# kiyo-masui/bitshuffle

Measured on AMD Instinct MI355X. Metric: device-resident GiB/s bitshuffle+LZ4 encode+decode, 4 GiB int16; % HBM roofline, higher is better.
Workload: dtype u8; 1 GPU; bitshuffle+LZ4 encode+decode round trip, 4 GiB int16 G1 correlated noise per GPU, default blocks (4096 elem), device-resident, decoder rebuilds the block index; elem_size=2, block_size=4096, bytes_per_gpu=4294967296, compressed_bytes_rank0=1813937762, parallelism=shard-per-gpu x1

## Files before the change

### bitshuffle_amd/csrc/bshuf_dev.h

```cpp
#pragma once

#include <hip/hip_runtime.h>
#include <stdint.h>

namespace bshuf {

constexpr int kWave = 64;

constexpr int kBlockedMult = 8;
constexpr int kMinMatch = 4;
constexpr int kMfLimit = 12;
constexpr int kLastLiterals = 5;
constexpr int kLz4MinLength = kMfLimit + 1;
constexpr int kU16TableLimit = 65536 + kMfLimit - 1;
constexpr uint32_t kMaxDistance = 65535;

__host__ __device__ inline int lz4_bound(int n) { return n + n / 255 + 16; }

struct Layout {
    int64_t nfull;
    int32_t bs;
    int32_t last;
    int32_t E;
    int64_t nblocks() const { return nfull + (last ? 1 : 0); }
};

// ... 157 lines not shown
    } else {
#pragma unroll
        for (int i = 0; i < EK / 2; i++) {
            const u32x4 v = *(const gbl128c*)(p + 16 * i);
            w[4 * i + 0] = v.x;
            w[4 * i + 1] = v.y;
            w[4 * i + 2] = v.z;
            w[4 * i + 3] = v.w;
        }
    }
}

template <int EK>
__device__ __forceinline__ void store_group(uint8_t* p, const uint32_t (&w)[2 * EK]) {
    if constexpr (EK == 1) {
        *(gbl64*)p = u32x2{w[0], w[1]};
    } else {
#pragma unroll
        for (int i = 0; i < EK / 2; i++)
            *(gbl128*)(p + 16 * i) = u32x4{w[4 * i + 0], w[4 * i + 1], w[4 * i + 2], w[4 * i + 3]};
    }
}

#ifndef BSHUF_TICKET_SHARDS
#define BSHUF_TICKET_SHARDS 8
#endif
constexpr int kTicketShards = BSHUF_TICKET_SHARDS;
constexpr int kTicketStride = 16;
static_assert((kTicketShards & (kTicketShards - 1)) == 0, "shards: a power of two");

struct Tickets {
    uint32_t* ctr;
    int64_t base;
    __device__ __forceinline__ Tickets(uint32_t* set, int64_t first)
        : ctr(set ? set + (blockIdx.x & (kTicketShards - 1)) * kTicketStride : nullptr),
          base(set ? first + gridDim.x + (blockIdx.x & (kTicketShards - 1)) : (int64_t)gridDim.x) {}
    __device__ __forceinline__ uint32_t request(int lane, uint32_t n = 1u) const {
        uint32_t t = 0;
        if (ctr && lane == 0) t = __hip_atomic_fetch_add(ctr, n, __ATOMIC_RELAXED, __HIP_MEMORY_SCOPE_AGENT);
        return t;
    }
    __device__ __forceinline__ int64_t block(uint32_t t, int64_t last, uint32_t k = 0u) const {
        if (!ctr) return last + base;
        const uint32_t v = (uint32_t)__builtin_amdgcn_readfirstlane((int)t) + k;
        return base + (int64_t)kTicketShards * (int64_t)v;
    }
};

}
```

### bitshuffle_amd/csrc/enc_common.h

```cpp
#pragma once

#include "launch.h"

namespace bshuf {

struct EncArgs {
    const uint8_t* in;
    uint8_t* scratch;
    uint64_t* foot;
    int64_t slot;
    Layout L;
    int32_t desc_ok;
    int32_t desc_off;
    const Seg* segs;
    const uint32_t* blk_seg;
    int32_t raw8;
    int64_t blk0;
    uint32_t* tickets;
};

template <int EK>
struct BlockRegs {
    static constexpr int kIters = EK ? 8192 / (kWave * 8 * EK) : 1;
    uint32_t w[kIters][2 * (EK ? EK : 1)];
};

template <int EK>
__device__ __forceinline__ void issue_block_loads(BlockRegs<EK>& R, const uint8_t* src, int P,
                                                  int lane) {
#pragma unroll
    for (int it = 0; it < BlockRegs<EK>::kIters; it++) {
        const int g = it * kWave + lane;
        if (g < P) load_group<EK>(src + (int64_t)g * 8 * EK, R.w[it]);
    }
}

template <int EK>
__device__ __forceinline__ void transpose_regs_to_lds(const BlockRegs<EK>& R, lds8* D, int P,
                                                      int g0, int lane) {
#pragma unroll
    for (int it = 0; it < BlockRegs<EK>::kIters; it++) {
// ... 103 lines not shown
```

### bitshuffle_amd/csrc/launch.h

```cpp
#pragma once

#include <hip/hip_runtime.h>
#include <stddef.h>
#include <stdint.h>

#include <algorithm>

#include "bshuf_dev.h"

namespace bshuf {

bool prof_on();
class ProfScope {
  public:
    ProfScope(const char* name, hipStream_t s);
    ~ProfScope();

  private:
    const char* name_;
    hipStream_t s_;
    void* a_;
};

int tuning_variant();
#ifdef BSHUF_DIAG
int diag_variant();
#endif

constexpr int kPipeSegs = 8;
constexpr int64_t kPipeMinBlocks = 65536;
constexpr int kPipeEvents = kPipeSegs + 2;
constexpr int kNoPipe = 1 << 20;
struct PipeCtx {
    hipStream_t side = nullptr;
    hipEvent_t ev[kPipeEvents] = {};
};
PipeCtx* pipe_ctx(hipStream_t s);
hipError_t stream_after(hipStream_t s, hipStream_t from, hipEvent_t ev);

constexpr size_t kTicketSetBytes = (size_t)kTicketShards * kTicketStride * sizeof(uint32_t);
constexpr int kEncTicketSets = kPipeSegs;
constexpr int kStaticSched = 1 << 24;
constexpr int kTicketSched = 1 << 25;
enum TicketKernel { kTicketsEncode, kTicketsDecode };
bool ticket_sched(TicketKernel k, int64_t block_bytes);

int64_t persistent_grid(const void* fn, int threads, size_t lds, int64_t work);
hipError_t dev_fill(void* p, int v, size_t n, hipStream_t s);
hipError_t stage_upload(const void* host, size_t bytes, void* dev, hipStream_t s);

struct Seg {
    const uint8_t* in;
    uint8_t* out;
    int64_t first;
    int64_t nfull;
    int64_t tail;
    int64_t in_nbytes;
    int64_t chunk0;
    int64_t nchunks;
    int64_t seq0;
    int64_t* result;
    int32_t last;
    int32_t pad_;
};

hipError_t launch_seg_map(const Seg* segs, int nsegs, uint32_t* map, bool chunks, hipStream_t s);

constexpr int kTileGroups = 256;
// ... 75 lines not shown
```

### bitshuffle_amd/csrc/lz4_decode.hip

```cpp
#include <hipcub/hipcub.hpp>

#include <cstdlib>

#include "launch.h"
#include "lds_copy.h"
#include "lz4_scan.h"

namespace bshuf {

namespace {

constexpr int64_t kAmbiguous = -2;
constexpr int64_t kDead = -1;
constexpr int kIdxWinMax = 32768;
constexpr int kIdxCandCap = 512;

#ifdef BSHUF_DIAG
constexpr int kDDiagCopies = 64;
__device__ unsigned long long g_ddiag[kDDiagCopies * 16];
__device__ unsigned long long g_ddiag_bw[4] = {~0ull, 0, 0, 0};
struct DDiag {
    uint64_t t, acc[8];
    uint32_t cnt[8];
    __device__ DDiag() : t(__builtin_amdgcn_s_memtime()) {
        for (int i = 0; i < 8; i++) acc[i] = 0, cnt[i] = 0;
    }
    __device__ __forceinline__ void stamp(int i) {
        const uint64_t n = __builtin_amdgcn_s_memtime();
        acc[i] += n - t;
        t = n;
    }
    __device__ __forceinline__ void count(int i, uint32_t v) { cnt[i] += v; }
    __device__ void flush(int lane) {
        if (lane == 0)
            for (int i = 0; i < 8; i++) {
                atomicAdd(&g_ddiag[(blockIdx.x % kDDiagCopies) * 16 + i], (unsigned long long)acc[i]);
                atomicAdd(&g_ddiag[(blockIdx.x % kDDiagCopies) * 16 + 8 + i], (unsigned long long)cnt[i]);
            }
        if (lane == 0) {
            atomicMin(&g_ddiag_bw[0], (unsigned long long)cnt[3]);
            atomicMax(&g_ddiag_bw[1], (unsigned long long)cnt[3]);
            atomicAdd(&g_ddiag_bw[2], (unsigned long long)cnt[3]);
            atomicAdd(&g_ddiag_bw[3], 1ull);
// ... 552 lines not shown
        }
        dg.stamp(2);
    }
}

struct DecArgs {
    const uint8_t* in;
    int64_t in_nbytes;
    const uint64_t* offs;
    uint8_t* out;
    int64_t* status;
    long long* bad;
    Layout L;
    uint32_t maxlen;
    int32_t cap;
    uint32_t* seq;
    const Seg* segs;
    const uint32_t* blk_seg;
    int32_t stage_off;
    int32_t ip_end;
    int64_t blk0, blk1;
    const int64_t* dlen;
    uint32_t* tickets;
};

__device__ __forceinline__ void resolve_len(DecArgs& a) {
    if (a.dlen) {
        a.in_nbytes = readable_bytes(*a.dlen, a.in_nbytes);
        a.dlen = nullptr;
    }
}

struct BlockLoc {
    const uint8_t* in;
    int64_t in_nbytes;
    uint8_t* out;
    uint32_t* seq;
    long long* bad;
    int m;
    bool last;
};

__device__ __forceinline__ BlockLoc block_loc(const DecArgs& a, int64_t k, int64_t nb, uint32_t s) {
    BlockLoc b;
    if (!a.segs) {
        b.in = a.in;
// ... 369 lines not shown
    }
    const gbl128c* g4 = span_base(a, sp);
    const int nch = span_chunks(a, sp);
    for (int c = lane; c < nch; c += kWave) ((lds128*)Cbuf)[c] = g4[c];
    return sp.loc.seq[sp.o0 / 3 + lane];
}

template <int EK, int VAR>
__global__ __launch_bounds__(64) __attribute__((amdgpu_waves_per_eu((VAR & 512) ? (EK == 0 ? 4 : 5) : 1)))
void k_lz4_decode(DecArgs a, int64_t nb) {
    extern __shared__ __attribute__((aligned(16))) uint8_t smem[];
    const int lane = threadIdx.x;
    const int E = EK ? EK : a.L.E;
    lds8* D = to_lds(smem);
    lds8* Cbuf = to_lds(smem) + a.cap + 16;
    constexpr bool kG = (VAR & 16) != 0;
    constexpr bool kIP = (VAR & 512) != 0;
    auto cbuf_of = [&](const Span& sp) -> lds8* {
        return kIP ? to_lds(smem) + a.ip_end - 16 * span_chunks(a, sp) : Cbuf;
    };
    int64_t blk = a.blk0 + blockIdx.x;
    const int64_t end = a.blk1;
    if (blk >= end) return;
    const Tickets tks(a.tickets, a.blk0);
    const uint32_t tk0 = tks.request(lane, 2u);
    uint32_t tk = tks.request(lane);
    resolve_len(a);

    PayRegsT<kIP ? kPayItersIP : kPayIters> R;
    auto fits = [&](const Span& sp) { return kIP || span_fits(a, sp); };
    Span cur = span_from(a, issue_offs(a, blk, nb, lane), nb);
    uint32_t cur_pos;
    if constexpr (kG) {
        cur_pos = cur.loc.seq[cur.o0 / 3 + lane];
    } else {
        const bool in_regs = fits(cur);
        if (in_regs) issue_pay(R, a, cur, lane);
        cur_pos = land_record(R, in_regs, a, cur, cbuf_of(cur), lane);
    }
    int64_t next = tks.block(tk0, blk);
    int64_t nn = tks.block(tk0, next, 1u);
    Span nxt = {};
    bool nxt_in_regs = false;
    uint32_t pref_pos = 0;
    constexpr bool kTouch = (VAR & 32) != 0;
    Touch t_cur{0u, 0u}, t_nxt{0u, 0u}, t_nxt2{0u, 0u};
    if (next < end) {
        nxt = span_from(a, issue_offs(a, next, nb, lane), nb);
        if constexpr (kG) {
            pref_pos = nxt.loc.seq[nxt.o0 / 3 + lane];
            if constexpr (kTouch) t_nxt = touch_record(nxt, lane);
        } else {
            nxt_in_regs = fits(nxt);
            if (nxt_in_regs) issue_pay(R, a, nxt, lane);
        }
    }
    OffRegs O{0, 0};
    if (nn < end) O = issue_offs(a, nn, nb, lane);
    int64_t n3 = end;
    auto offs_ahead = [&]() {
        n3 = tks.block(tk, nn);
        if (n3 < end) {
            tk = tks.request(lane);
            O = issue_offs(a, n3, nb, lane);
        }
    };
    __builtin_amdgcn_fence(__ATOMIC_RELEASE, "wavefront");
    __builtin_amdgcn_wave_barrier();
    DDiag dg;

    for (;;) {
        dg.stamp(5);
        const int P = cur.loc.m / 8;
        const int cp = span_shift(a, cur);
        lds8* const CB = cbuf_of(cur);
        const lds8* C = CB + cp;
        int status = 0, clen = 0;
        if (cur.scan < 0) {
            status = (int)cur.scan;
        } else if constexpr (kG) {
            if constexpr (kTouch) touch_done(t_cur);
            const uint8_t* rec = cur.loc.in + cur.o0;
            clen = (int)be32_global(rec);
            const uintptr_t b0 = (uintptr_t)(rec + 4);
// ... 147 lines not shown
                    nxt2_in_regs = fits(nxt2);
                    if (nxt2_in_regs) issue_pay(R, a, nxt2, lane);
                }
            }
        }
        __builtin_amdgcn_fence(__ATOMIC_RELEASE, "wavefront");
        __builtin_amdgcn_wave_barrier();
        dg.stamp(4);
        dg.count(3, 1);
        if (next >= end) break;
        blk = next;
        cur = nxt;
        cur_pos = nxt_pos;
        next = nn;
        nn = n3;
        nxt = nxt2;
        nxt_in_regs = nxt2_in_regs;
        if constexpr (kTouch) {
            t_cur = t_nxt;
            t_nxt = t_nxt2;
        }
    }
    dg.flush(lane);
}

__global__ __launch_bounds__(256) void k_decode_finish(const int64_t* __restrict__ status,
                                                       const uint64_t* __restrict__ offs,
                                                       int64_t nblocks, const long long* bad,
                                                       const int64_t* idx_err, const uint8_t* in,
                                                       int64_t in_nbytes, uint8_t* tail_dst,
                                                       int64_t tail, int64_t* result,
                                                       const int64_t* dlen) {
    if (dlen) {
        const int64_t d = *dlen;
        if (d < 0) {
            if (threadIdx.x == 0) *result = d;
            return;
        }
        in_nbytes = readable_bytes(d, in_nbytes);
    }
    const long long last_bad = *bad;
    const int64_t end = nblocks ? (int64_t)offs[nblocks - 1] + status[nblocks - 1] : 0;
    const bool idx_bad = idx_err && *idx_err != 0;
    const bool ok = last_bad < 0 && !idx_bad && end + tail <= in_nbytes;
    if (ok)
        for (int64_t i = threadIdx.x; i < tail; i += blockDim.x) tail_dst[i] = in[end + i];
// ... 258 lines not shown
            if (diag_variant() == 64) fn = BSHUF_DEC(4, 576);
            if (diag_variant() == 72) fn = BSHUF_DEC(4, 584);
#endif
            break;
        case 8: fn = inplace ? BSHUF_DEC(8, 512) : touch ? BSHUF_DEC(8, 48) : (grec ? BSHUF_DEC(8, 16) : BSHUF_DEC(8, 0)); break;
        default: fn = inplace ? BSHUF_DEC(0, 512) : touch ? BSHUF_DEC(0, 48) : (grec ? BSHUF_DEC(0, 16) : BSHUF_DEC(0, 0)); break;
    }
#undef BSHUF_DEC
    hipError_t e = hipSuccess;
#if defined(BSHUF_DIAG) || defined(BSHUF_OCC)
    if (const char* w = getenv("BSHUF_DIAG_DEC_WAVES")) {
        const size_t want = (size_t)(160 * 1024 / atoi(w)) & ~(size_t)1023;
        if (want > lds) lds = want;
    }
#endif
    if (lds > 65536) {
        e = hipFuncSetAttribute(fn, hipFuncAttributeMaxDynamicSharedMemorySize, (int)lds);
        if (e != hipSuccess) return e;
    }
    auto dec = [&](int64_t f0, int64_t f1, hipStream_t st) -> hipError_t {
        DecArgs aa = a;
        aa.blk0 = f0;
        aa.blk1 = f1;
        const dim3 grid((unsigned)persistent_grid(fn, kWave, lds, f1 - f0));
        ProfScope prof("k_lz4_decode", st);
        void* args[] = {&aa, const_cast<int64_t*>(&nb)};
        hipError_t r = hipLaunchKernel(fn, grid, dim3(kWave), args, lds, st);
        return r != hipSuccess ? r : hipGetLastError();
    };
    a.blk0 = 0;
    a.blk1 = nb;
    if (!ticket_sched(kTicketsDecode, (int64_t)L.bs * L.E) || nb >= ((int64_t)1 << 31)) a.tickets = nullptr;
    e = scan_impl(a, nb, s);
    return e != hipSuccess ? e : dec(0, nb, s);
}

__global__ void k_seg_dlen(Seg* __restrict__ segs, const int64_t* __restrict__ dlens, int nsegs) {
    const int i = (int)(blockIdx.x * blockDim.x + threadIdx.x);
    if (i < nsegs) segs[i].in_nbytes = readable_bytes(dlens[i], segs[i].in_nbytes);
}

__global__ __launch_bounds__(64) void k_decode_finish_batch(const int64_t* __restrict__ status,
                                                            const uint64_t* __restrict__ offs,
                                                            const long long* bad,
                                                            const int64_t* idx_err, const Seg* segs,
                                                            int32_t bs, int32_t E, const int64_t* dlens) {
// ... 66 lines not shown
    ProfScope prof("k_decode_finish", s);
    hipLaunchKernelGGL(k_decode_finish_batch, dim3((unsigned)nsegs), dim3(64), 0, s, b.status, b.offs,
                       (const long long*)b.bad, (const int64_t*)b.idx_err, segs, L.bs, L.E, dlens);
    return hipGetLastError();
}

}

#ifdef BSHUF_DIAG
extern "C" int bshuf_diag_read_dec(unsigned long long* out) {
    static unsigned long long all[bshuf::kDDiagCopies * 16];
    if (hipMemcpyFromSymbol(all, HIP_SYMBOL(bshuf::g_ddiag), sizeof all) != hipSuccess) return -1;
    for (int i = 0; i < 16; i++) {
        out[i] = 0;
        for (int c = 0; c < bshuf::kDDiagCopies; c++) out[i] += all[c * 16 + i];
    }
    static const unsigned long long bw0[4] = {~0ull, 0, 0, 0};
    if (hipMemcpyFromSymbol(out + 16, HIP_SYMBOL(bshuf::g_ddiag_bw), sizeof bw0) != hipSuccess ||
        hipMemcpyToSymbol(HIP_SYMBOL(bshuf::g_ddiag_bw), bw0, sizeof bw0) != hipSuccess)
        return -1;
    static const unsigned long long z[bshuf::kDDiagCopies * 16] = {0};
    return hipMemcpyToSymbol(HIP_SYMBOL(bshuf::g_ddiag), z, sizeof z) == hipSuccess ? 0 : -1;
}
#endif
```

### bitshuffle_amd/csrc/lz4_encode.hip

```cpp
#include <hipcub/hipcub.hpp>

#include <atomic>
#include <type_traits>
#include <cstdlib>
#include <mutex>

#include "enc_common.h"
#include "launch.h"
#include "lds_copy.h"

namespace bshuf {

namespace {

constexpr int kTableBytes = 16384;

#ifdef BSHUF_DIAG
constexpr int kDiagCopies = 64;
__device__ unsigned long long g_diag[kDiagCopies * 32];
#define DIAG_DECL                                   \
    uint64_t _dt = __builtin_amdgcn_s_memtime();    \
    uint64_t _acc[8] = {0, 0, 0, 0, 0, 0, 0, 0};    \
    uint32_t _cnt[8] = {0, 0, 0, 0, 0, 0, 0, 0};
#define STAMP(i)                                       \
    do {                                               \
        const uint64_t _n = __builtin_amdgcn_s_memtime(); \
        _acc[i] += _n - _dt;                           \
        _dt = _n;                                      \
    } while (0)
#define COUNT(i, v) (_cnt[i] += (v))
#define DIAG_FLUSH                                                          \
    do {                                                                    \
        if (lane == 0)                                                      \
            for (int _i = 0; _i < 8; _i++) {                                \
                atomicAdd(&g_diag[(blockIdx.x % kDiagCopies) * 32 + _i],   \
                          (unsigned long long)_acc[_i]);                    \
                atomicAdd(&g_diag[(blockIdx.x % kDiagCopies) * 32 + 8 + _i], \
                          (unsigned long long)_cnt[_i]);                    \
            }                                                               \
    } while (0)
__device__ unsigned long long g_diag_bw[4] = {~0ull, 0, 0, 0};
#define KDIAG_DECL                                   \
    uint64_t _kt = __builtin_amdgcn_s_memtime();     \
    uint64_t _kacc[4] = {0, 0, 0, 0};                \
    unsigned long long _kblocks = 0;
#define KBLOCK (++_kblocks)
#define KSTAMP(i)                                       \
    do {                                                \
        const uint64_t _n = __builtin_amdgcn_s_memtime(); \
        _kacc[i] += _n - _kt;                           \
        _kt = _n;                                       \
    } while (0)
#define KDIAG_FLUSH                                                                     \
    do {                                                                                \
        if (lane == 0)                                                                  \
            for (int _i = 0; _i < 4; _i++)                                              \
                atomicAdd(&g_diag[(blockIdx.x % kDiagCopies) * 32 + 16 + _i], _kacc[_i]); \
        if (lane == 0) {                                                                \
            atomicMin(&g_diag_bw[0], _kblocks);                                         \
            atomicMax(&g_diag_bw[1], _kblocks);                                         \
            atomicAdd(&g_diag_bw[2], _kblocks);                                         \
            atomicAdd(&g_diag_bw[3], 1ull);                                             \
        }                                                                               \
    } while (0)
// ... 1500 lines not shown
}
__device__ __forceinline__ void raw_to_lds(const RawRegs& R, lds8* S, int nbytes, int lane) {
#pragma unroll
    for (int it = 0; it < kRawIters; it++) {
        const int i = it * kWave + lane;
        if (8 * i < nbytes) ((lds64v*)S)[i] = u32x2{R.w[it].x, R.w[it].y};
    }
}

#ifndef BSHUF_FLUSH4
#define BSHUF_FLUSH4 1
#endif
template <int EK, bool WIDE, int VAR>
__global__ __launch_bounds__(64) void k_lz4_encode(EncArgs a, int64_t nb) {
    extern __shared__ __attribute__((aligned(16))) uint8_t smem[];
    __builtin_amdgcn_s_setprio(2);
    const int lane = threadIdx.x;
    const int E = EK ? EK : a.L.E;
    (void)smem;
    lds8* const L0 = lds_origin();
    lds8* D = L0 + kTableBytes;
    int64_t blk = blockIdx.x;
    if (blk >= nb) return;
    const Tickets tks(a.tickets, 0);
    uint32_t tk = tks.request(lane);
    constexpr bool kBatch = (VAR & 256) != 0;
    auto blk_m = [&](int64_t k) {
        if (!kBatch) return k < a.L.nfull ? a.L.bs : a.L.last;
        const Seg& g = a.segs[a.blk_seg[k + a.blk0]];
        return k + a.blk0 - g.first < g.nfull ? a.L.bs : g.last;
    };
    auto blk_src = [&](int64_t k) {
        if (!kBatch) return a.in + k * (int64_t)a.L.bs * E;
        const Seg& g = a.segs[a.blk_seg[k + a.blk0]];
        return g.in + (k + a.blk0 - g.first) * (int64_t)a.L.bs * E;
    };

    BlockRegs<EK> R;
    BlockRegs4<EK> R4;
    RawRegs RW;
    auto raw_fits = [&](int m) { return EK == 0 && a.raw8 && m * E <= kRawBytes; };
    constexpr bool kX4 = (VAR & 4) == 0;
    constexpr bool kReadback = (VAR & 128) != 0;
    constexpr int kRegGroups = BlockRegs<EK>::kIters * kWave;
    constexpr int kRegGroups4 = BlockRegs4<EK>::kIters * kWave * 4;
    auto fits = [&](int m) { return EK != 0 && m / 8 <= kRegGroups; };
    auto fits4 = [&](int m) { return kX4 && EK != 0 && (m / 8) % 4 == 0 && m / 8 <= kRegGroups4; };
    if constexpr (EK != 0) {
// ... 92 lines not shown
#pragma unroll
                    for (int it = 0; it < BlockRegs<EK>::kIters; it++) {
                        const int g = g0 + it * kWave + lane;
                        if (g < P) load_group<EK>(src + (int64_t)g * 8 * EK, T.w[it]);
                    }
                    transpose_regs_to_lds<EK>(T, D, P, g0, lane);
                }
            }
        } else {
            for (int i = lane; i < P * E; i += kWave) {
                const int g = i / E, b = i - g * E;
                uint64_t v = 0;
#pragma unroll
                for (int k = 0; k < 8; k++)
                    v |= (uint64_t)src[(int64_t)(8 * g + k) * E + b] << (8 * k);
                v = tr8x8(v);
#pragma unroll
                for (int j = 0; j < 8; j++) D[(8 * b + j) * P + g] = (uint8_t)(v >> (8 * j));
            }
        }
        __builtin_amdgcn_fence(__ATOMIC_RELEASE, "wavefront");
        __builtin_amdgcn_wave_barrier();
        const int64_t next = tks.block(tk, blk);
        if (next < nb) tk = tks.request(lane);
        if constexpr (kDefer) {
            flush_pending();
            if constexpr (kFlush4) {
#pragma unroll
                for (int k = 0; k < kTableBytes / 16 / kWave; k++)
                    ((lds128*)L0)[k * kWave + lane] = u32x4{0u, 0u, 0u, 0u};
            } else {
                for (int i = lane; i < kTableBytes / 16; i += kWave)
                    ((lds128*)L0)[i] = u32x4{0u, 0u, 0u, 0u};
            }
            __builtin_amdgcn_fence(__ATOMIC_RELEASE, "wavefront");
            __builtin_amdgcn_wave_barrier();
        }
        if constexpr (EK != 0) {
            if (next < nb) {
                const int mn = blk_m(next);
                if (fits4(mn))
                    issue_block_loads4<EK>(R4, blk_src(next), mn / 8, lane);
                else if (fits(mn))
                    issue_block_loads<EK>(R, blk_src(next), mn / 8, lane);
            }
        } else {
// ... 34 lines not shown
                    }
                } else {
                    for (int i = lane; i < kTableBytes / 16; i += kWave)
                        ((lds128*)L0)[i] = u32x4{0u, 0u, 0u, 0u};
                    __builtin_amdgcn_fence(__ATOMIC_RELEASE, "wavefront");
                    __builtin_amdgcn_wave_barrier();
                }
            }
        }
        if (c < 0) {
            EmitBytes<> em{out + 4, D, lane};
            c = lz4_encode_block<WIDE, kReadback, (VAR & (8 | 512 | 2048))>(D, n, T, em, lane);
            if (lane < 4) out[lane] = (uint8_t)((uint32_t)c >> (24 - 8 * lane));
        }
        if (lane == 0 && pend_blk != blk) a.foot[blk] = 4 + (uint64_t)c;
        __builtin_amdgcn_fence(__ATOMIC_RELEASE, "wavefront");
        __builtin_amdgcn_wave_barrier();
        KSTAMP(2);
        if (next >= nb) break;
        blk = next;
    }
    if constexpr (kDefer) flush_pending();
    KDIAG_FLUSH;
}

constexpr int kCompactPerWg = 4;
constexpr int kCompactUnroll = 4;

__device__ __forceinline__ u32x4 pair_bytes(const u32x4 a, const u32x4 b, int t) {
    const uint32_t w[8] = {a.x, a.y, a.z, a.w, b.x, b.y, b.z, b.w};
    const uint32_t sh = (uint32_t)(t & 3);
    u32x4 v;
    switch (t >> 2) {
#define BSHUF_PAIR(D)                                                                          \
    case D:                                                                                     \
        v = u32x4{__builtin_amdgcn_alignbyte(w[D + 1], w[D], sh),                               \
                  __builtin_amdgcn_alignbyte(w[D + 2], w[D + 1], sh),                           \
                  __builtin_amdgcn_alignbyte(w[D + 3], w[D + 2], sh),                           \
                  __builtin_amdgcn_alignbyte(w[D + 4], w[D + 3], sh)};                          \
        break;
        BSHUF_PAIR(0)
        BSHUF_PAIR(1)
        BSHUF_PAIR(2)
        default: BSHUF_PAIR(3)
#undef BSHUF_PAIR
    }
// ... 298 lines not shown
                         const EncodeBufs& b, int64_t* d_result, hipStream_t s, bool fast) {
    const int64_t nb = L.nblocks();
    hipError_t e = fill_foot_end(b, nb, s);
    if (e != hipSuccess) return e;
    fast = fast && (int64_t)L.bs * L.E <= kFastMaxBlockBytes;
    if (nb > 0 && (int64_t)L.bs * L.E > max_lds_encode_bytes()) {
        e = launch_encode_large(in, L, b, b.shuf, b.tables, s);
        if (e != hipSuccess) return e;
    } else if (nb > 0) {
        const int64_t nmax = (int64_t)L.bs * L.E;
        const bool wide = nmax >= kU16TableLimit;
        const bool desc = !wide && 4 + lz4_bound((int)nmax) + 15 <= kTableBytes;
        const int32_t desc_off = (int32_t)(((nmax + 15) & ~15) + kDataPad);
        EncArgs a{in, b.scratch, b.foot, b.slot, L, desc ? 1 : 0, desc_off, nullptr, nullptr,
                  ((uintptr_t)in & 7) == 0 ? 1 : 0};
        const size_t lds = kTableBytes + (size_t)desc_off + (desc ? kDescBytes : 0);
        const bool wide_last = L.last && (int64_t)L.last * L.E >= kU16TableLimit;
        const bool aligned = ((uintptr_t)in & 15) == 0;
        const int ek = aligned && (L.E == 1 || L.E == 2 || L.E == 4 || L.E == 8) ? L.E : 0;
        auto go = [&](Layout LL, bool w, int64_t count, int64_t first, int set) -> hipError_t {
            EncArgs aa = a;
            aa.L = LL;
            aa.tickets = ticket_set(b, L, nb, set);
            aa.in = a.in + first * (int64_t)L.bs * L.E;
            aa.scratch = a.scratch + first * b.slot;
            aa.foot = a.foot + first;
            aa.L.nfull = LL.nfull - first;
            if (fast) return launch_encode_fast(aa, count, ek, s);
#define BSHUF_E(EKV)                                                         \
    case EKV:                                                                \
        return w ? launch_enc_t<EKV, true>(aa, count, lds, s)                \
                 : launch_enc_t<EKV, false>(aa, count, lds, s);
            switch (ek) {
                BSHUF_E(0)
                BSHUF_E(1)
                BSHUF_E(2)
                BSHUF_E(4)
                BSHUF_E(8)
            }
#undef BSHUF_E
            return hipErrorInvalidValue;
        };
        PipeCtx* pc = (wide == wide_last || !L.last) && nb >= kPipeMinBlocks ? pipe_ctx(s) : nullptr;
        if (pc) return encode_pipelined(nb, s, pc, b, [&](int64_t f0, int64_t f1, int set) {
            return go(L, wide, f1 - f0, f0, set);
        }, out, nullptr, nullptr, nullptr, [&](hipStream_t st) {
// ... 40 lines not shown
    const int64_t nb = L.nfull;
    hipError_t e = fill_foot_end(b, nb, s);
    if (e != hipSuccess) return e;
    fast = fast && (int64_t)L.bs * L.E <= kFastMaxBlockBytes;
    if (nb > 0) {
        const int64_t nmax = (int64_t)L.bs * L.E;
        const bool wide = nmax >= kU16TableLimit;
        for (int i = 0; i < nsegs; i++)
            if (hsegs[i].last && ((int64_t)hsegs[i].last * L.E >= kU16TableLimit) != wide)
                return hipErrorInvalidValue;
        const bool desc = !wide && 4 + lz4_bound((int)nmax) + 15 <= kTableBytes;
        const int32_t desc_off = (int32_t)(((nmax + 15) & ~15) + kDataPad);
        bool raw8 = true;
        for (int i = 0; i < nsegs; i++) raw8 = raw8 && ((uintptr_t)hsegs[i].in & 7) == 0;
        EncArgs a{nullptr, b.scratch, b.foot, b.slot, L, desc ? 1 : 0, desc_off, segs, blk_seg,
                  raw8 ? 1 : 0};
        const size_t lds = kTableBytes + (size_t)desc_off + (desc ? kDescBytes : 0);
        bool aligned = true;
        for (int i = 0; i < nsegs; i++) aligned = aligned && ((uintptr_t)hsegs[i].in & 15) == 0;
        const int ek = aligned && (L.E == 1 || L.E == 2 || L.E == 4 || L.E == 8) ? L.E : 0;
        auto go = [&](int64_t f0, int64_t f1, int set) -> hipError_t {
            EncArgs aa = a;
            aa.tickets = ticket_set(b, L, nb, set);
            aa.blk0 = f0;
            aa.scratch = a.scratch + f0 * b.slot;
            aa.foot = a.foot + f0;
            const int64_t cnt = f1 - f0;
            if (fast) return launch_encode_fast(aa, cnt, ek, s);
#define BSHUF_E(EKV)                                                                  \
    case EKV:                                                                         \
        return wide ? launch_enc_t<EKV, true, 256>(aa, cnt, lds, s)                   \
                    : launch_enc_t<EKV, false, 256>(aa, cnt, lds, s);
            switch (ek) {
                BSHUF_E(0)
                BSHUF_E(1)
                BSHUF_E(2)
                BSHUF_E(4)
                BSHUF_E(8)
            }
#undef BSHUF_E
            return hipErrorInvalidValue;
        };
        PipeCtx* pc = nb >= kPipeMinBlocks ? pipe_ctx(s) : nullptr;
        if (pc) return encode_pipelined(nb, s, pc, b, go, nullptr, segs, blk_seg, block_offsets,
                                        [&](hipStream_t st) {
            ProfScope prof("k_encode_finish", st);
// ... 34 lines not shown
hipError_t launch_seg_map(const Seg* segs, int nsegs, uint32_t* map, bool chunks, hipStream_t s) {
    if (nsegs <= 0) return hipSuccess;
    hipLaunchKernelGGL(k_seg_map, dim3((unsigned)nsegs), dim3(256), 0, s, segs, map, chunks ? 1 : 0);
    return hipGetLastError();
}

}

#ifdef BSHUF_DIAG
extern "C" int bshuf_diag_read(unsigned long long* out) {
    static unsigned long long all[bshuf::kDiagCopies * 32];
    if (hipMemcpyFromSymbol(all, HIP_SYMBOL(bshuf::g_diag), sizeof all) != hipSuccess) return -1;
    for (int i = 0; i < 32; i++) {
        out[i] = 0;
        for (int c = 0; c < bshuf::kDiagCopies; c++) out[i] += all[c * 32 + i];
    }
    static const unsigned long long bw0[4] = {~0ull, 0, 0, 0};
    if (hipMemcpyFromSymbol(out + 20, HIP_SYMBOL(bshuf::g_diag_bw), sizeof bw0) != hipSuccess ||
        hipMemcpyToSymbol(HIP_SYMBOL(bshuf::g_diag_bw), bw0, sizeof bw0) != hipSuccess)
        return -1;
    static const unsigned long long z[bshuf::kDiagCopies * 32] = {0};
    return hipMemcpyToSymbol(HIP_SYMBOL(bshuf::g_diag), z, sizeof z) == hipSuccess ? 0 : -1;
}
#endif
```

### bitshuffle_amd/csrc/prof.hip

```cpp
#include <hip/hip_runtime.h>

#include <algorithm>
#include <stdio.h>
#include <stdlib.h>
#include <string.h>

#include <map>
#include <mutex>
#include <string>
#include <vector>

#include "launch.h"

namespace bshuf {

namespace {

struct Rec {
    const char* name;
    hipEvent_t a, b;
};

struct Prof {
    std::mutex mu;
// ... 3 lines not shown
    std::vector<hipEvent_t> pool;
    hipEvent_t get() {
        if (!pool.empty()) {
            hipEvent_t e = pool.back();
            pool.pop_back();
            return e;
        }
        hipEvent_t e = nullptr;
        (void)hipEventCreate(&e);
        return e;
    }
};

Prof& P() {
    static Prof* p = new Prof();
    return *p;
}

}

bool prof_on() { return P().on; }

static thread_local int t_variant = 0;
int tuning_variant() { return t_variant & ~(kNoPipe | kStaticSched | kTicketSched); }
constexpr int64_t kDecodeTicketMinBlock = 2048;
bool ticket_sched(TicketKernel k, int64_t block_bytes) {
    if (t_variant & kStaticSched) return false;
    if (t_variant & kTicketSched) return true;
    return k == kTicketsEncode || block_bytes >= kDecodeTicketMinBlock;
}

namespace {
constexpr int kPipeDevices = 16;
struct PipeSet {
    PipeCtx c[kPipeDevices];
    bool bad[kPipeDevices] = {};
    ~PipeSet() {
        for (PipeCtx& x : c) {
            if (!x.side) continue;
            (void)hipStreamSynchronize(x.side);
            for (hipEvent_t& e : x.ev)
                if (e) (void)hipEventDestroy(e);
            (void)hipStreamDestroy(x.side);
        }
    }
};
thread_local PipeSet t_pipe;
}

PipeCtx* pipe_ctx(hipStream_t s) {
    if (t_variant & kNoPipe) return nullptr;
    hipStreamCaptureStatus cap = hipStreamCaptureStatusNone;
// ... 63 lines not shown
    if (!p.on) return;
    std::lock_guard<std::mutex> g(p.mu);
    if (!p.only.empty() && p.only != name) return;
    a_ = p.get();
    (void)hipEventRecord((hipEvent_t)a_, s);
}

ProfScope::~ProfScope() {
    if (!a_) return;
    Prof& p = P();
    std::lock_guard<std::mutex> g(p.mu);
    hipEvent_t b = p.get();
    (void)hipEventRecord(b, s_);
    p.recs.push_back(Rec{name_, (hipEvent_t)a_, b});
}

}

using namespace bshuf;

extern "C" {

int bshuf_set_variant(int v) {
    const int vv = v & ~(kNoPipe | kStaticSched | kTicketSched);
    if (vv != 0 && vv != 2 && vv != 4 && vv != 8 && vv != 16 && vv != 32 && vv != 64 && vv != 128 && vv != 512 && vv != 1024 && vv != 2048 && vv != 4096 && vv != 8192 && vv != 16384 && vv != 24576 && vv != 40960 && vv != 57344 && vv != 65536 && vv != 319488 &&
        vv != 172032 && vv != 450560 &&
        vv != 2793472 && vv != 3072000)
        return -71;
    t_variant = v;
    return 0;
}

#ifdef BSHUF_DIAG
void bshuf_diag_set_ablation(int v) { g_diag_variant = v; }
#endif

void bshuf_prof_enable(int on) {
    Prof& p = P();
    std::lock_guard<std::mutex> g(p.mu);
    p.on = on != 0;
    if (p.on) {
        const size_t want = 4096 + p.recs.size() * 2;
        while (p.pool.size() < want) {
            hipEvent_t e = nullptr;
            if (hipEventCreate(&e) != hipSuccess) break;
            p.pool.push_back(e);
        }
// ... 41 lines not shown
```

### bitshuffle_amd/csrc/scan_host.cpp

```cpp
#include <stdint.h>

#include "lz4_scan.h"

namespace {
struct HostReader {
    const uint8_t* P;
    uint32_t operator()(int p) const { return P[p]; }
};
struct HostOut {
    uint32_t* pos;
    void put(int i, uint32_t v, int op) {
        pos[i] = v;
        (void)op;
    }
};
}

extern "C" int bshuf_hostcheck_scan(const uint8_t* payload, int clen, int n, uint32_t* pos,
                                    int* nseq) {
    HostReader rd{payload};
    HostOut out{pos};
    int cnt = 0;
    const int r = bshuf::scan_block(rd, clen, n, out, cnt);
    *nseq = cnt;
    return r;
}
```

Before: 325.9 GiB/s.

## Add cross-shard ticket stealing to encoder persistent-kernel scheduler

Extends the sharded atomic ticket scheduler so a wave whose home shard is exhausted reads the other shards' counters and steals blocks from the shard with the most remaining work. The intent is to shrink the tail imbalance where some shards finish early while others still hold blocks. It is enabled by default for the encoder when the block is at least 1 KiB, and the decoder uses a non-stealing instantiation. The cost is extra atomic loads and readlane work at the end of each shard, plus some counter overdraw. Diagnostics for per-shard own and stolen counts are added behind a compile flag.

```diff
diff --git a/bitshuffle_amd/csrc/bshuf_dev.h b/bitshuffle_amd/csrc/bshuf_dev.h
--- a/bitshuffle_amd/csrc/bshuf_dev.h
+++ b/bitshuffle_amd/csrc/bshuf_dev.h
@@ -2,6 +2,8 @@
 
 #include <hip/hip_runtime.h>
 #include <stdint.h>
+
+#include "ticket_steal.h"
 
 namespace bshuf {
 
@@ -205,29 +207,130 @@
     }
 }
 
-#ifndef BSHUF_TICKET_SHARDS
-#define BSHUF_TICKET_SHARDS 8
+constexpr int kTicketStride = 16;
+constexpr int64_t kTicketMaxWaves = 4608;
+constexpr int64_t kTicketOverdraw = kTicketMaxWaves * (3 + kTicketShards);
+static_assert(((int64_t)1 << 31) / kTicketShards + 1 + kTicketOverdraw < ((int64_t)1 << 32),
+              "32-bit counters cover every nb < 2^31");
+
+struct Ticket {
+    uint32_t t;
+    int shard;
+};
+
+template <bool STEAL>
+struct TicketsT {
+    uint32_t* set;
+    int64_t g0;
+    int64_t end;
+    int shard;
+    uint32_t dead;
+    bool steal;
+    __device__ __forceinline__ TicketsT(uint32_t* s, int64_t first, int64_t e, bool st)
+        : set(s),
+          g0(s ? first + gridDim.x : (int64_t)gridDim.x),
+          end(e),
+          shard((int)(blockIdx.x & (kTicketShards - 1))),
+          dead(0u),
+          steal(STEAL && st && kTicketShards > 1) {}
+    __device__ __forceinline__ Ticket request(int lane, uint32_t n = 1u) const {
+        uint32_t t = 0;
+        if (set && lane == 0)
+            t = __hip_atomic_fetch_add(set + shard * kTicketStride, n, __ATOMIC_RELAXED, __HIP_MEMORY_SCOPE_AGENT);
+        return Ticket{t, shard};
+    }
+    __device__ __forceinline__ int64_t block(const Ticket& q, int64_t last, uint32_t k = 0u) {
+        if (!set) return last + g0;
+        if constexpr (!STEAL) {
+            const uint32_t v = (uint32_t)__builtin_amdgcn_readfirstlane((int)q.t) + k;
+            return g0 + shard + (int64_t)kTicketShards * (int64_t)v;
+        }
+        if (__builtin_amdgcn_readfirstlane(q.shard) == shard) {
+            const uint32_t v = (uint32_t)__builtin_amdgcn_readfirstlane((int)q.t) + k;
+            const int64_t b = g0 + shard + (int64_t)kTicketShards * (int64_t)v;
+            if (b < end || !steal) return b;
+        }
+        return uni64(steal_block());
+    }
+    static __device__ __forceinline__ int64_t uni64(int64_t x) {
+        const uint32_t lo = (uint32_t)__builtin_amdgcn_readfirstlane((int)(uint32_t)x);
+        const uint32_t hi = (uint32_t)__builtin_amdgcn_readfirstlane((int)(uint32_t)((uint64_t)x >> 32));
+        return (int64_t)(((uint64_t)hi << 32) | lo);
+    }
+    __device__ __forceinline__ int64_t steal_block() {
+        const int lane = threadIdx.x;
+#pragma unroll 1
+        for (int i = 0; i < kTicketShards; i++) {
+            uint32_t left = 0;
+            if (lane < kTicketShards) {
+                const uint32_t drawn =
+                    __hip_atomic_load(set + lane * kTicketStride, __ATOMIC_RELAXED, __HIP_MEMORY_SCOPE_AGENT);
+                left = ticket_remaining(ticket_limit(g0, 0, end, lane), drawn);
+            }
+            uint32_t rem[kTicketShards];
+#pragma unroll
+            for (int c = 0; c < kTicketShards; c++)
+                rem[c] = (dead >> c) & 1u ? 0u : (uint32_t)__builtin_amdgcn_readlane((int)left, c);
+            const int victim = __builtin_amdgcn_readfirstlane(ticket_victim(rem, shard));
+            if (victim < 0) break;
+            uint32_t t = 0;
+            if (lane == 0)
+                t = __hip_atomic_fetch_add(set + victim * kTicketStride, 1u, __ATOMIC_RELAXED,
+                                           __HIP_MEMORY_SCOPE_AGENT);
+            const uint32_t v = (uint32_t)__builtin_amdgcn_readfirstlane((int)t);
+            const int64_t b = g0 + victim + (int64_t)kTicketShards * (int64_t)v;
+            if (b < end) {
+                shard = victim;
+                return b;
+            }
+            dead |= 1u << victim;
+        }
+        return end;
+    }
+};
+
+using Tickets = TicketsT<true>;
+
+#ifdef BSHUF_DIAG
+constexpr int kShardDiagSlots = 16;
+constexpr int kShardDiagWords = 5;
+constexpr int kShardDiagSize = kShardDiagSlots * kTicketShards * kShardDiagWords;
+struct ShardDiag {
+    uint64_t t0;
+    uint32_t own = 1, stolen = 0;
+    int home;
+    __device__ __forceinline__ ShardDiag()
+        : t0(__builtin_amdgcn_s_memrealtime()), home((int)(blockIdx.x & (kTicketShards - 1))) {}
+    template <bool STEAL>
+    __device__ __forceinline__ void drew(const TicketsT<STEAL>& t, int64_t b) {
+        if (b >= t.end) return;
+        if (t.shard == home) own++;
+        else stolen++;
+    }
+    __device__ __forceinline__ void flush(unsigned long long* g, int slot, int lane) const {
+        if (lane != 0) return;
+        unsigned long long* p = g + ((slot % kShardDiagSlots) * kTicketShards + home) * kShardDiagWords;
+        atomicMin(p + 0, (unsigned long long)t0);
+        atomicMax(p + 1, (unsigned long long)__builtin_amdgcn_s_memrealtime());
+        atomicAdd(p + 2, (unsigned long long)own);
+        atomicAdd(p + 3, (unsigned long long)stolen);
+        atomicAdd(p + 4, stolen ? 1ull : 0ull);
+    }
+};
+template <class Sym>
+inline int shard_diag_read(const Sym& sym, unsigned long long* out) {
+    static unsigned long long init[kShardDiagSize];
+    if (hipMemcpyFromSymbol(out, sym, sizeof init) != hipSuccess) return -1;
+    for (int i = 0; i < kShardDiagSize; i++) init[i] = i % kShardDiagWords == 0 ? ~0ull : 0ull;
+    return hipMemcpyToSymbol(sym, init, sizeof init) == hipSuccess ? 0 : -1;
+}
+#define SHARD_DIAG_DECL ShardDiag _sd
+#define SHARD_DIAG_DREW(t, b) _sd.drew(t, b)
+#define SHARD_DIAG_FLUSH(g, slot, lane) _sd.flush(g, slot, lane)
+#else
+#define SHARD_DIAG_DECL ((void)0)
+#define SHARD_DIAG_DREW(t, b) ((void)0)
+#define SHARD_DIAG_FLUSH(g, slot, lane) ((void)0)
 #endif
-constexpr int kTicketShards = BSHUF_TICKET_SHARDS;
-constexpr int kTicketStride = 16;
-static_assert((kTicketShards & (kTicketShards - 1)) == 0, "shards: a power of two");
-
-struct Tickets {
-    uint32_t* ctr;
-    int64_t base;
-    __device__ __forceinline__ Tickets(uint32_t* set, int64_t first)
-        : ctr(set ? set + (blockIdx.x & (kTicketShards - 1)) * kTicketStride : nullptr),
-          base(set ? first + gridDim.x + (blockIdx.x & (kTicketShards - 1)) : (int64_t)gridDim.x) {}
-    __device__ __forceinline__ uint32_t request(int lane, uint32_t n = 1u) const {
-        uint32_t t = 0;
-        if (ctr && lane == 0) t = __hip_atomic_fetch_add(ctr, n, __ATOMIC_RELAXED, __HIP_MEMORY_SCOPE_AGENT);
-        return t;
-    }
-    __device__ __forceinline__ int64_t block(uint32_t t, int64_t last, uint32_t k = 0u) const {
-        if (!ctr) return last + base;
-        const uint32_t v = (uint32_t)__builtin_amdgcn_readfirstlane((int)t) + k;
-        return base + (int64_t)kTicketShards * (int64_t)v;
-    }
-};
-
-}
+
+}
diff --git a/bitshuffle_amd/csrc/enc_common.h b/bitshuffle_amd/csrc/enc_common.h
--- a/bitshuffle_amd/csrc/enc_common.h
+++ b/bitshuffle_amd/csrc/enc_common.h
@@ -17,6 +17,10 @@
     int32_t raw8;
     int64_t blk0;
     uint32_t* tickets;
+    int32_t steal;
+#ifdef BSHUF_DIAG
+    int32_t diag_slot;
+#endif
 };
 
 template <int EK>
diff --git a/bitshuffle_amd/csrc/launch.h b/bitshuffle_amd/csrc/launch.h
--- a/bitshuffle_amd/csrc/launch.h
+++ b/bitshuffle_amd/csrc/launch.h
@@ -42,8 +42,10 @@
 constexpr int kEncTicketSets = kPipeSegs;
 constexpr int kStaticSched = 1 << 24;
 constexpr int kTicketSched = 1 << 25;
+constexpr int kNoSteal = 1 << 26;
 enum TicketKernel { kTicketsEncode, kTicketsDecode };
 bool ticket_sched(TicketKernel k, int64_t block_bytes);
+bool ticket_steal(int64_t block_bytes);
 
 int64_t persistent_grid(const void* fn, int threads, size_t lds, int64_t work);
 hipError_t dev_fill(void* p, int v, size_t n, hipStream_t s);
diff --git a/bitshuffle_amd/csrc/lz4_decode.hip b/bitshuffle_amd/csrc/lz4_decode.hip
--- a/bitshuffle_amd/csrc/lz4_decode.hip
+++ b/bitshuffle_amd/csrc/lz4_decode.hip
@@ -19,6 +19,8 @@
 constexpr int kDDiagCopies = 64;
 __device__ unsigned long long g_ddiag[kDDiagCopies * 16];
 __device__ unsigned long long g_ddiag_bw[4] = {~0ull, 0, 0, 0};
+__device__ unsigned long long g_ddiag_shard[kShardDiagSize];
+int g_ddiag_launches = 0;
 struct DDiag {
     uint64_t t, acc[8];
     uint32_t cnt[8];
@@ -617,6 +619,9 @@
     int64_t blk0, blk1;
     const int64_t* dlen;
     uint32_t* tickets;
+#ifdef BSHUF_DIAG
+    int32_t diag_slot;
+#endif
 };
 
 __device__ __forceinline__ void resolve_len(DecArgs& a) {
@@ -1032,9 +1037,10 @@
     int64_t blk = a.blk0 + blockIdx.x;
     const int64_t end = a.blk1;
     if (blk >= end) return;
-    const Tickets tks(a.tickets, a.blk0);
-    const uint32_t tk0 = tks.request(lane, 2u);
-    uint32_t tk = tks.request(lane);
+    TicketsT<false> tks(a.tickets, a.blk0, end, false);
+    const Ticket tk0 = tks.request(lane, 2u);
+    Ticket tk = tks.request(lane);
+    SHARD_DIAG_DECL;
     resolve_len(a);
 
     PayRegsT<kIP ? kPayItersIP : kPayIters> R;
@@ -1049,7 +1055,9 @@
         cur_pos = land_record(R, in_regs, a, cur, cbuf_of(cur), lane);
     }
     int64_t next = tks.block(tk0, blk);
+    SHARD_DIAG_DREW(tks, next);
     int64_t nn = tks.block(tk0, next, 1u);
+    SHARD_DIAG_DREW(tks, nn);
     Span nxt = {};
     bool nxt_in_regs = false;
     uint32_t pref_pos = 0;
@@ -1070,6 +1078,7 @@
     int64_t n3 = end;
     auto offs_ahead = [&]() {
         n3 = tks.block(tk, nn);
+        SHARD_DIAG_DREW(tks, n3);
         if (n3 < end) {
             tk = tks.request(lane);
             O = issue_offs(a, n3, nb, lane);
@@ -1263,6 +1272,7 @@
         }
     }
     dg.flush(lane);
+    SHARD_DIAG_FLUSH(g_ddiag_shard, a.diag_slot, lane);
 }
 
 __global__ __launch_bounds__(256) void k_decode_finish(const int64_t* __restrict__ status,
@@ -1567,6 +1577,9 @@
         DecArgs aa = a;
         aa.blk0 = f0;
         aa.blk1 = f1;
+#ifdef BSHUF_DIAG
+        aa.diag_slot = g_ddiag_launches++;
+#endif
         const dim3 grid((unsigned)persistent_grid(fn, kWave, lds, f1 - f0));
         ProfScope prof("k_lz4_decode", st);
         void* args[] = {&aa, const_cast<int64_t*>(&nb)};
@@ -1679,4 +1692,9 @@
     static const unsigned long long z[bshuf::kDDiagCopies * 16] = {0};
     return hipMemcpyToSymbol(HIP_SYMBOL(bshuf::g_ddiag), z, sizeof z) == hipSuccess ? 0 : -1;
 }
+extern "C" int bshuf_diag_read_shards_dec(unsigned long long* out) {
+    const int n = bshuf::g_ddiag_launches;
+    bshuf::g_ddiag_launches = 0;
+    return bshuf::shard_diag_read(HIP_SYMBOL(bshuf::g_ddiag_shard), out) == 0 ? n : -1;
+}
 #endif
diff --git a/bitshuffle_amd/csrc/lz4_encode.hip b/bitshuffle_amd/csrc/lz4_encode.hip
--- a/bitshuffle_amd/csrc/lz4_encode.hip
+++ b/bitshuffle_amd/csrc/lz4_encode.hip
@@ -40,6 +40,8 @@
             }                                                               \
     } while (0)
 __device__ unsigned long long g_diag_bw[4] = {~0ull, 0, 0, 0};
+__device__ unsigned long long g_diag_shard[kShardDiagSize];
+int g_diag_launches = 0;
 #define KDIAG_DECL                                   \
     uint64_t _kt = __builtin_amdgcn_s_memtime();     \
     uint64_t _kacc[4] = {0, 0, 0, 0};                \
@@ -1586,8 +1588,9 @@
     lds8* D = L0 + kTableBytes;
     int64_t blk = blockIdx.x;
     if (blk >= nb) return;
-    const Tickets tks(a.tickets, 0);
-    uint32_t tk = tks.request(lane);
+    Tickets tks(a.tickets, 0, nb, a.steal != 0);
+    Ticket tk = tks.request(lane);
+    SHARD_DIAG_DECL;
     constexpr bool kBatch = (VAR & 256) != 0;
     auto blk_m = [&](int64_t k) {
         if (!kBatch) return k < a.L.nfull ? a.L.bs : a.L.last;
@@ -1726,6 +1729,7 @@
         __builtin_amdgcn_fence(__ATOMIC_RELEASE, "wavefront");
         __builtin_amdgcn_wave_barrier();
         const int64_t next = tks.block(tk, blk);
+        SHARD_DIAG_DREW(tks, next);
         if (next < nb) tk = tks.request(lane);
         if constexpr (kDefer) {
             flush_pending();
@@ -1806,6 +1810,7 @@
     }
     if constexpr (kDefer) flush_pending();
     KDIAG_FLUSH;
+    SHARD_DIAG_FLUSH(g_diag_shard, a.diag_slot, lane);
 }
 
 constexpr int kCompactPerWg = 4;
@@ -2150,6 +2155,10 @@
             EncArgs aa = a;
             aa.L = LL;
             aa.tickets = ticket_set(b, L, nb, set);
+            aa.steal = ticket_steal((int64_t)L.bs * L.E) ? 1 : 0;
+#ifdef BSHUF_DIAG
+            aa.diag_slot = g_diag_launches++;
+#endif
             aa.in = a.in + first * (int64_t)L.bs * L.E;
             aa.scratch = a.scratch + first * b.slot;
             aa.foot = a.foot + first;
@@ -2236,6 +2245,10 @@
         auto go = [&](int64_t f0, int64_t f1, int set) -> hipError_t {
             EncArgs aa = a;
             aa.tickets = ticket_set(b, L, nb, set);
+            aa.steal = ticket_steal((int64_t)L.bs * L.E) ? 1 : 0;
+#ifdef BSHUF_DIAG
+            aa.diag_slot = g_diag_launches++;
+#endif
             aa.blk0 = f0;
             aa.scratch = a.scratch + f0 * b.slot;
             aa.foot = a.foot + f0;
@@ -2316,4 +2329,9 @@
     static const unsigned long long z[bshuf::kDiagCopies * 32] = {0};
     return hipMemcpyToSymbol(HIP_SYMBOL(bshuf::g_diag), z, sizeof z) == hipSuccess ? 0 : -1;
 }
+extern "C" int bshuf_diag_read_shards(unsigned long long* out) {
+    const int n = bshuf::g_diag_launches;
+    bshuf::g_diag_launches = 0;
+    return bshuf::shard_diag_read(HIP_SYMBOL(bshuf::g_diag_shard), out) == 0 ? n : -1;
+}
 #endif
diff --git a/bitshuffle_amd/csrc/prof.hip b/bitshuffle_amd/csrc/prof.hip
--- a/bitshuffle_amd/csrc/prof.hip
+++ b/bitshuffle_amd/csrc/prof.hip
@@ -49,12 +49,18 @@
 bool prof_on() { return P().on; }
 
 static thread_local int t_variant = 0;
-int tuning_variant() { return t_variant & ~(kNoPipe | kStaticSched | kTicketSched); }
+int tuning_variant() { return t_variant & ~(kNoPipe | kStaticSched | kTicketSched | kNoSteal); }
 constexpr int64_t kDecodeTicketMinBlock = 2048;
 bool ticket_sched(TicketKernel k, int64_t block_bytes) {
     if (t_variant & kStaticSched) return false;
     if (t_variant & kTicketSched) return true;
     return k == kTicketsEncode || block_bytes >= kDecodeTicketMinBlock;
+}
+constexpr int64_t kStealMinBlock = 1024;
+bool ticket_steal(int64_t block_bytes) {
+    if (t_variant & kNoSteal) return false;
+    if (t_variant & kTicketSched) return true;
+    return block_bytes >= kStealMinBlock;
 }
 
 namespace {
@@ -164,7 +170,7 @@
 extern "C" {
 
 int bshuf_set_variant(int v) {
-    const int vv = v & ~(kNoPipe | kStaticSched | kTicketSched);
+    const int vv = v & ~(kNoPipe | kStaticSched | kTicketSched | kNoSteal);
     if (vv != 0 && vv != 2 && vv != 4 && vv != 8 && vv != 16 && vv != 32 && vv != 64 && vv != 128 && vv != 512 && vv != 1024 && vv != 2048 && vv != 4096 && vv != 8192 && vv != 16384 && vv != 24576 && vv != 40960 && vv != 57344 && vv != 65536 && vv != 319488 &&
         vv != 172032 && vv != 450560 &&
         vv != 2793472 && vv != 3072000)
diff --git a/bitshuffle_amd/csrc/scan_host.cpp b/bitshuffle_amd/csrc/scan_host.cpp
--- a/bitshuffle_amd/csrc/scan_host.cpp
+++ b/bitshuffle_amd/csrc/scan_host.cpp
@@ -1,6 +1,7 @@
 #include <stdint.h>
 
 #include "lz4_scan.h"
+#include "ticket_steal.h"
 
 namespace {
 struct HostReader {
@@ -25,3 +26,16 @@
     *nseq = cnt;
     return r;
 }
+
+extern "C" int bshuf_hostcheck_ticket_shards(void) { return bshuf::kTicketShards; }
+extern "C" int64_t bshuf_hostcheck_ticket_limit(int64_t first, int64_t G, int64_t end, int shard) {
+    return bshuf::ticket_limit(first, G, end, shard);
+}
+extern "C" uint32_t bshuf_hostcheck_ticket_remaining(int64_t limit, uint32_t drawn) {
+    return bshuf::ticket_remaining(limit, drawn);
+}
+extern "C" int bshuf_hostcheck_ticket_victim(const uint32_t* remaining, int own) {
+    uint32_t r[bshuf::kTicketShards];
+    for (int c = 0; c < bshuf::kTicketShards; c++) r[c] = remaining[c];
+    return bshuf::ticket_victim(r, own);
+}
diff --git a/bitshuffle_amd/csrc/ticket_steal.h b/bitshuffle_amd/csrc/ticket_steal.h
--- /dev/null
+++ b/bitshuffle_amd/csrc/ticket_steal.h
@@ -0,0 +1,42 @@
+#pragma once
+#include <stdint.h>
+
+#if defined(__HIPCC__)
+#define BSHUF_TS_HD __host__ __device__
+#else
+#define BSHUF_TS_HD
+#endif
+
+#ifndef BSHUF_TICKET_SHARDS
+#define BSHUF_TICKET_SHARDS 8
+#endif
+
+namespace bshuf {
+
+constexpr int kTicketShards = BSHUF_TICKET_SHARDS;
+static_assert((kTicketShards & (kTicketShards - 1)) == 0, "shards: a power of two");
+
+BSHUF_TS_HD inline int64_t ticket_limit(int64_t first, int64_t G, int64_t end, int c) {
+    const int64_t left = end - (first + G + c);
+    return left <= 0 ? 0 : (left + kTicketShards - 1) / kTicketShards;
+}
+
+BSHUF_TS_HD inline uint32_t ticket_remaining(int64_t limit, uint32_t drawn) {
+    return (int64_t)drawn >= limit ? 0u : (uint32_t)(limit - (int64_t)drawn);
+}
+
+BSHUF_TS_HD inline int ticket_victim(const uint32_t (&remaining)[kTicketShards], int own) {
+    int best = -1, best_dist = kTicketShards;
+    uint32_t most = 0;
+    for (int c = 0; c < kTicketShards; c++) {
+        const int dist = (c - own - 1) & (kTicketShards - 1);
+        if (remaining[c] > most || (remaining[c] == most && most != 0 && dist < best_dist)) {
+            most = remaining[c];
+            best = c;
+            best_dist = dist;
+        }
+    }
+    return best;
+}
+
+}
```

After: 336.9 GiB/s (median of 6 runs). 3.4% higher.
